# SKA-INAF/caesar-mrcnn

Hardware: AMD Instinct MI355X
Metric: train images/sec (whole node) + detect ms/image, ResNet-101 256x256 (higher is better)
Workload: dtype f32; 1 GPU; resnet101+FPN 256x256 3-class (+bg), nimg_per_gpu=4, train step (fwd+bwd+SGD), 512 train ROIs, 2000 proposals; global_batch=4, parallelism=dp1, weights=random init (Keras defaults)

## Files before the change

caesar-mrcnn_amd/_hip.py:

```python
import ctypes as C
import os
import threading

PKG_DIR = os.path.dirname(os.path.abspath(__file__))
LIB_PATH = os.path.join(PKG_DIR, "libmrcnn_hip.so")


class HipPathError(RuntimeError):
    pass


class ConvDesc(C.Structure):
    _fields_ = [(n, C.c_int32) for n in (
        "N", "H", "W", "Cin", "Cout", "KH", "KW", "stride", "pad_t", "pad_l", "OH", "OW",
        "act", "res_mode", "out_mode", "cmod")] + [
        ("out_n_stride", C.c_int64), ("out_h_stride", C.c_int64), ("out_w_stride", C.c_int64)]


class ConvProblem(C.Structure):
    _fields_ = [("d", ConvDesc)] + [(n, C.c_void_p) for n in ("x", "w", "bias", "scale", "shift", "res", "out", "z_out")]


class WgradProblem(C.Structure):
    _fields_ = [("d", ConvDesc), ("x", C.c_void_p), ("dy", C.c_void_p), ("dw", C.c_void_p), ("accumulate", C.c_int32)]
# ... 203 lines not shown
    "mrcnn_cast_to_h16": (C.c_int, [_P, _P, C.c_int64, C.c_int, C.c_float, _P]),
    "mrcnn_epilogue_bwd_h16": (C.c_int, [C.c_int] + [_P] * 10 + [C.c_int64, C.c_int, C.c_int, C.c_float, _P]),
    "mrcnn_epilogue_bwd_h16_dy": (C.c_int, [C.c_int] + [_P] * 11 + [C.c_int64, C.c_int, C.c_int, C.c_float, _P]),
    "mrcnn_cast_from_h16": (C.c_int, [_P, _P, C.c_int64, C.c_int, C.c_float, _P]),
    "mrcnn_axpy_from_h16": (C.c_int, [_P, _P, C.c_int64, C.c_int, C.c_float, _P]),
    "mrcnn_rpn_targets_workspace": (C.c_size_t, [C.POINTER(RpnTargetDesc)]),
    "mrcnn_rpn_targets": (C.c_int, [C.POINTER(RpnTargetDesc)] + [_P] * 7 + [C.c_size_t, _P]),
    "mrcnn_detection_workspace": (C.c_size_t, [C.POINTER(DetectionDesc)]),
    "mrcnn_detection_fwd": (C.c_int, [C.POINTER(DetectionDesc)] + [_P] * 6 + [C.c_size_t, _P]),
    "mrcnn_losses_workspace": (C.c_size_t, [C.POINTER(LossDesc)]),
    "mrcnn_losses_fwd_bwd": (C.c_int, [C.POINTER(LossDesc)] + [_P] * 18 + [C.c_size_t, _P]),
    "mrcnn_grad_prepare": (C.c_int, [_P, _P, C.c_float, _P, C.c_int64, _P, _P]),
    "mrcnn_sumsq": (C.c_int, [_P, C.c_int64, _P, _P]),
    "mrcnn_sgd_momentum": (C.c_int, [_P, _P, _P, _P, C.c_float, C.c_float, C.c_float, _P, C.c_int64, _P]),
    "mrcnn_sgd_momentum_guarded": (C.c_int, [_P, _P, _P, _P, C.c_float, C.c_float, C.c_float, _P, C.c_int64, _P, _P]),
    "mrcnn_winograd_buffer_floats": (C.c_size_t, [C.c_int, C.c_int, C.c_int, C.c_int, C.c_int]),
    "mrcnn_winograd_weights": (C.c_int, [_P, _P, C.c_int, C.c_int, C.c_int, _P]),
    "mrcnn_gemm_batched_f32": (C.c_int, [_P, _P, _P, C.c_int, C.c_int, C.c_int, C.c_int, _P]),
    "mrcnn_winograd_gemm": (C.c_int, [_P, _P, _P, C.c_int, C.c_int, C.c_int, C.c_int, _P]),
    "mrcnn_winograd_group_floats": (C.c_size_t, [C.POINTER(WinoGroup), C.c_int, C.c_int]),
    "mrcnn_winograd_input_g": (C.c_int, [_P, _P, C.c_int, C.c_int, C.c_int, C.c_int, C.POINTER(WinoGroup), _P]),
    "mrcnn_winograd_weights_g": (C.c_int, [_P, _P, C.c_int, C.c_int, C.c_int, C.c_int, _P]),
    "mrcnn_winograd_output_g": (C.c_int, [_P, _P, _P, _P, _P, _P, C.c_int, C.c_int, C.c_int, C.c_int, C.c_int, C.POINTER(WinoGroup), _P]),
    "mrcnn_winograd_output_bwd_rows": (C.c_int, [C.POINTER(WinoGroup), C.c_int, C.c_int]),
    "mrcnn_winograd_output_bwd_g": (C.c_int, [_P] * 8 + [C.c_int, C.c_int, C.c_int, C.c_int, C.c_int, C.POINTER(WinoGroup), _P]),
    "mrcnn_winograd_output_bwd_zmask_g": (C.c_int, [_P] * 8 + [C.c_int, C.c_int, C.c_int, C.c_int, C.POINTER(WinoGroup), _P]),
    "mrcnn_winograd_output_bwd_sums": (C.c_int, [_P, C.c_int, C.c_int, _P, _P, _P, _P]),
    "mrcnn_winograd_dy_g": (C.c_int, [_P, _P, C.c_int, C.c_int, C.c_int, C.c_int, C.POINTER(WinoGroup), _P]),
    "mrcnn_winograd_dw_g": (C.c_int, [_P, _P, C.c_int, C.c_int, C.c_int, C.c_int, C.c_int, _P]),
    "mrcnn_deconv2x2_gemm": (C.c_int, [_P, _P, _P, _P, C.c_int, C.c_int, C.c_int, C.c_int, C.c_int, C.c_int, _P]),
    "mrcnn_allreduce_load": (C.c_int, [C.c_char_p]),
    "mrcnn_allreduce_unique_id": (C.c_int, [_P]),
    "mrcnn_allreduce_init": (C.c_int, [C.POINTER(_P), _P, C.c_int, C.c_int]),
    "mrcnn_allreduce_scratch": (C.c_size_t, [C.c_int, C.c_int64, C.c_int]),
    "mrcnn_allreduce_grad": (C.c_int, [_P, _P, C.c_int64, C.c_int64, C.c_int, _P, C.c_size_t, _P]),
    "mrcnn_allreduce_direct_plan": (C.c_int, [C.c_int, C.c_int, C.c_int64, C.c_int64, C.c_int, _P, _P, _P, _P]),
    "mrcnn_allreduce_direct_simulate": (C.c_int, [_P, _P, C.c_size_t, C.c_int, C.c_int64, C.c_int64, _P]),
    "mrcnn_allreduce_destroy": (C.c_int, [_P]),
    "mrcnn_allreduce_last_error": (C.c_char_p, []),
    "mrcnn_tuning_set": (C.c_int, [C.c_char_p, C.c_longlong]),
    "mrcnn_hip_version": (C.c_char_p, []),
}

_lib = None
_proxy = None
_tape = None
# ... 119 lines not shown
```

caesar-mrcnn_amd/csrc/winograd.hip:

```cpp
#include "common.h"
#include <type_traits>
#include <string.h>

template <int CV> struct WinoVec;
template <> struct WinoVec<4> { typedef f32x4 type; };
template <> struct WinoVec<2> { typedef float type __attribute__((ext_vector_type(2))); };

template <int OT, typename V> __device__ __forceinline__ void wino_bt(const V (&d)[OT + 2], V (&t)[OT + 2]) {
    if constexpr (OT == 2) {
        t[0] = d[0] - d[2];
        t[1] = d[1] + d[2];
        t[2] = d[2] - d[1];
        t[3] = d[1] - d[3];
    } else {
        const V a = d[4] - 4.f * d[2], b = d[3] - 4.f * d[1], c = d[4] - d[2], e = 2.f * (d[3] - d[1]);
        t[0] = 4.f * d[0] - 5.f * d[2] + d[4];
        t[1] = a + b;
        t[2] = a - b;
        t[3] = c + e;
        t[4] = c - e;
        t[5] = 4.f * d[1] - 5.f * d[3] + d[5];
    }
}
template <int OT, typename V> __device__ __forceinline__ void wino_at(const V (&m)[OT + 2], V (&y)[OT]) {
// ... 181 lines not shown
    const long long t = i / cn;
    const int c = (int)(i - t * cn) * CV;
    vec bi = {}, sc, sh = {};
#pragma unroll
    for (int e = 0; e < CV; ++e) sc[e] = 1.f;
    if (bias) bi = *(const vec*)(bias + c);
    if (scale) { sc = *(const vec*)(scale + c); sh = *(const vec*)(shift + c); }
    wino_output_tile<OTH, OTW, CV>(Mt, out, z, bi, sc, sh, H, W, C, Tp, act, g, t, c);
}

template <int CV>
__device__ __forceinline__ typename WinoVec<CV>::type wino_buffer_load(__amdgpu_buffer_rsrc_t rsrc, unsigned voff, unsigned soff) {
    typename WinoVec<CV>::type r;
    if constexpr (CV == 2) {
        const auto v = __builtin_amdgcn_raw_buffer_load_b64(rsrc, (int)voff, (int)soff, 0);
        r[0] = __uint_as_float(v[0]); r[1] = __uint_as_float(v[1]);
    } else {
        const auto v = __builtin_amdgcn_raw_buffer_load_b128(rsrc, (int)voff, (int)soff, 0);
        r[0] = __uint_as_float(v[0]); r[1] = __uint_as_float(v[1]); r[2] = __uint_as_float(v[2]); r[3] = __uint_as_float(v[3]);
    }
    return r;
}

template <int OTH, int OTW, int CV, int MASK>
__global__ __launch_bounds__(256) void winograd_output_bwd_kernel(const float* __restrict__ Mt, float* __restrict__ dz_out,
                                                                  const float* __restrict__ below_out, const float* __restrict__ below_z,
                                                                  const float* __restrict__ scale, const float* __restrict__ mean,
                                                                  const float* __restrict__ rstd, const float* __restrict__ fwd_shift,
                                                                  float* __restrict__ partials, int want_dg, int H, int W, int C, unsigned T,
                                                                  long long Tp, int lg, const WinoGrp g, const FastDiv d_th,
                                                                  const FastDiv d_tw) {
    typedef typename WinoVec<CV>::type vec;
    constexpr int ITH = OTH + 2, ITW = OTW + 2;
    __shared__ float sacc[3 * 4 * 256];
    const int L = 1 << lg, R = 256 >> lg;
    const int rsub = threadIdx.x >> lg, lane = threadIdx.x & (L - 1);
    const int c = lane * CV;
    vec sc, mu = {}, rs = {}, fsh = {};
#pragma unroll
    for (int e = 0; e < CV; ++e) sc[e] = 1.f;
    if (scale) sc = *(const vec*)(scale + c);
    if (want_dg) { mu = *(const vec*)(mean + c); rs = *(const vec*)(rstd + c); }
    if (MASK == 1) fsh = *(const vec*)(fwd_shift + c);
    const bool need_z = MASK == 1 || want_dg;
    vec a_db = {}, a_dg = {}, a_bias = {};
    const unsigned step = gridDim.x * (unsigned)R;
// ... 366 lines not shown
    if (!x || !V || !wino_grp_ok(g, N, H, W, C)) return MRCNN_ERR_ARG;
    const long long T = wino_grp_tiles(g, N);
    const WinoGrp k = {g->th_n, g->tw_n, g->oh0, g->ow0};
    const dim3 g4((unsigned)cdiv64(T * C / 4, 256)), g2((unsigned)cdiv64(T * C / 2, 256));
    WINO_LAUNCH_G(winograd_input_kernel, g, g4, g2, x, V, N, H, W, C, T, wino_rows(T), k);
    return mrcnn_launch_status();
}

extern "C" int mrcnn_winograd_weights_g(const float* w, float* U, int Cin, int Cout, int oth, int otw, void* stream) {
    if (!w || !U || Cin <= 0 || Cout <= 0 || (oth != 2 && oth != 4) || (otw != 2 && otw != 4)) return MRCNN_ERR_ARG;
    const dim3 grid((unsigned)cdiv64((long long)Cin * Cout, 256));
    WINO_LAUNCH_W(winograd_weight_kernel, oth, otw, grid, w, U, Cin, Cout);
    return mrcnn_launch_status();
}

extern "C" int mrcnn_winograd_output_g(const float* Mt, float* out, float* z, const float* bias, const float* scale, const float* shift,
                                       int N, int H, int W, int C, int act, const mrcnn_wino_group* g, void* stream) {
    if (!Mt || !out || !wino_grp_ok(g, N, H, W, C) || (scale && !shift)) return MRCNN_ERR_ARG;
    if (act != MRCNN_ACT_NONE && act != MRCNN_ACT_RELU) return MRCNN_ERR_UNSUPPORTED;
    const long long T = wino_grp_tiles(g, N);
    const WinoGrp k = {g->th_n, g->tw_n, g->oh0, g->ow0};
    const dim3 g4((unsigned)cdiv64(T * C / 4, 256)), g2((unsigned)cdiv64(T * C / 2, 256));
    WINO_LAUNCH_G(winograd_output_kernel, g, g4, g2, Mt, out, z, bias, scale, shift, N, H, W, C, T, wino_rows(T), act, k);
    return mrcnn_launch_status();
}

static int wino_bwd_lanes_lg(const mrcnn_wino_group* g, int C) {
    const int cn = C / wino_grp_cv(g);
    if (cn <= 0 || cn > 256 || (cn & (cn - 1)) || cn * wino_grp_cv(g) != C) return -1;
    int lg = 0;
    while ((1 << lg) < cn) ++lg;
    return lg;
}
extern "C" int mrcnn_winograd_output_bwd_rows(const mrcnn_wino_group* g, int N, int C) {
    if (!g || N <= 0 || (g->oth != 2 && g->oth != 4) || (g->otw != 2 && g->otw != 4) || g->th_n <= 0 || g->tw_n <= 0) return 0;
    const int lg = wino_bwd_lanes_lg(g, C);
    if (lg < 0) return 0;
    const long long T = wino_grp_tiles(g, N), R = 256 >> lg, cap = 4LL * mrcnn_num_cus();
    const long long wgs = cdiv64(T, R);
    return (int)(wgs < cap ? wgs : cap);
}

template <int MASK>
static int wino_output_bwd_launch(const float* Mt, float* dz_below, const float* below_out, const float* below_z, const float* scale,
                                  const float* mean, const float* rstd, const float* fwd_shift, float* partials, int N, int H, int W,
                                  int C, const mrcnn_wino_group* g, void* stream) {
// ... 117 lines not shown
```

caesar-mrcnn_amd/engine.py:

```python
import collections
import contextlib
import gc
import operator
from functools import partial
import os
import numpy as np
import torch

from . import ops
from . import _hip as _hip_mod
from ._hip import ACT_NONE, ACT_RELU, ACT_SIGMOID, RES_NONE, RES_SAME, RES_UP2
from .params import ParamLayout, deconv_gemm_to_keras, deconv_keras_to_gemm, granule_coefficients, init_weights

H16_WIDE_LAYERS = ("fpn_p2", "fpn_p3", "fpn_p4", "fpn_p5", "rpn_conv_shared", "mrcnn_class_conv1", "mrcnn_class_conv2")

LOSS_NAMES = ("rpn_class_loss", "rpn_bbox_loss", "mrcnn_class_loss", "mrcnn_bbox_loss", "mrcnn_mask_loss")


DIRECT, WINO, H16 = "direct", "winograd", "h16"
Ctx = collections.namedtuple("Ctx", "x z out act path V", defaults=(DIRECT, None))
BlockCtx = collections.namedtuple("BlockCtx", "a b c shortcut h16")


_on = lambda s: s != "0"

SWITCHES = (
    ("head_dtype", None, None, None, "ti"),
    ("sparse_mask_bwd", None, True, None, "t"),
    ("h16_wide", "MRCNN_H16_WIDE", True, _on, "ti"),
    ("h16_blocks", "MRCNN_H16_BLOCKS", True, _on, "ti"),
    ("h16_all_blocks", "MRCNN_H16_ALL_BLOCKS", True, _on, "ti"),
    ("h16_fused_bwd", "MRCNN_H16_FUSED_BWD", True, _on, "t"),
    ("h16_roialign", "MRCNN_H16_ROIALIGN", True, _on, "ti"),
    ("h16_phase_bwd", "MRCNN_H16_PHASE_BWD", True, _on, "t"),
    ("winograd", "MRCNN_WINOGRAD", True, _on, "ti"),
    ("winograd_wgrad", "MRCNN_WINOGRAD_WGRAD", True, _on, "t"),
    ("trunk_winograd", "MRCNN_WINOGRAD_TRUNK", True, _on, "ti"),
    ("trunk_winograd_min_rows", "MRCNN_WINOGRAD_TRUNK_MIN_ROWS", 4096, int, "ti"),
    ("infer_mask_tile", "MRCNN_WINOGRAD_INFER_MASK_TILE", 4, int, "i"),
    ("sk16_infer", "MRCNN_SK16_INFER", True, _on, "i"),
    ("fused_mask_out_bwd", None, True, None, "t"),
    ("fused_dgrad_epilogue", None, True, None, "t"),
    ("gather_roialign_bwd", "MRCNN_GATHER_ROIALIGN_BWD", True, _on, "t"),
    ("multi_launch", "MRCNN_MULTI_LAUNCH", True, _on, "ti"),
    ("wgrad_prio", "MRCNN_WGRAD_PRIO", 0, int, ""),
    ("aux_prio", "MRCNN_AUX_PRIO", 0, int, ""),
)
_TRAIN_SWITCHES = operator.attrgetter(*(s[0] for s in SWITCHES if "t" in s[4]))
_INFER_SWITCHES = operator.attrgetter(*(s[0] for s in SWITCHES if "i" in s[4]))
_INFER_CFG = operator.attrgetter("PRE_NMS_LIMIT", "POST_NMS_ROIS_INFERENCE", "RPN_NMS_THRESHOLD", "DETECTION_MAX_INSTANCES",
                                 "DETECTION_MIN_CONFIDENCE", "DETECTION_NMS_THRESHOLD")


@contextlib.contextmanager
def _capture(graph):
    gc.collect()
    was = gc.isenabled()
    gc.disable()
    try:
# ... 387 lines not shown
        x16 = ca.x
        N, H, W, C = x16.shape
        st = c2a.stride
        dz1 = self._h16_bwd(blk.c1, dy, c1c, S, need_dx=False)
        dx = ops.empty((N, H, W, C), x16.dtype, x16.device)
        strides = None
        if st != 1:
            ops.fill_zero(dx)
            strides = (H * W * C, st * W * C, st * C)
        self._h16_dgrad(blk.c1, dz1, out=dx, out_strides=strides)
        self._h16_dgrad(c2a, dza, dx_res=dx, out=dx, out_strides=strides)
        return dx

    def _S(self):
        return float(self.loss_scale) if self.head_dtype == torch.float16 else 1.0

    def _wino_fwd(self, op, x, act, train, infer_tile=2):
        out = ops.empty(tuple(x.shape[:3]) + (op.wshape[3],), torch.float32, x.device)
        z = ops.empty_like(out) if (train and op.bn) else None
        V = ops.empty((ops.winograd_v_floats(tuple(x.shape)),), torch.float32, x.device) if (train and self.winograd_wgrad) else None
        ops.conv2d_winograd(x, self._wino_U(op, 0, x.shape, train, infer_tile), op.b, op.scale, op.shift, act, out=out, z_out=z, keep_v=V)
        return out, (Ctx(x, z, out, act, WINO, V) if train else None)

    def _forward_multi(self, layers, xs, act=ACT_NONE, train=False):
        if self.trunk_winograd and any(self._wino_trunk_ok(op, x.shape) for op, x in zip(layers, xs)):
            res = [None] * len(layers)
            rest = []
            for i, (op, x) in enumerate(zip(layers, xs)):
                if self._wino_trunk_ok(op, x.shape):
                    res[i] = self._wino_fwd(op, x, act, train)
                else:
                    rest.append(i)
            if rest:
                sub = self._forward_multi([layers[i] for i in rest], [xs[i] for i in rest], act, train) if len(rest) > 1 else \
                    [layers[rest[0]].forward(xs[rest[0]], act, train=train)]
                for i, r in zip(rest, sub):
                    res[i] = r
            return res
        if self.multi_launch and 1 < len(layers) <= 5:
            probs, zs = [], []
            for op, x in zip(layers, xs):
                d = ops.conv_desc(tuple(x.shape), op.wshape, op.stride, op.padding, act)
                out = ops.empty((d.N, d.OH, d.OW, d.Cout), torch.float32, x.device)
                z = ops.empty_like(out) if (train and op.bn) else None
                zs.append(z)
                probs.append(dict(x=x, w=op.w, bias=op.b, scale=op.scale, shift=op.shift, stride=op.stride,
# ... 237 lines not shown
                x16 = ops.cast_to_h16(x, self.head_dtype)
            h1, c1 = self._h16_fwd(self.op("mrcnn_class_conv1"), x16, ACT_RELU, train)
            h2_16, c2 = self._h16_fwd(self.op("mrcnn_class_conv2"), h1, ACT_RELU, train)
            h2 = ops.cast_from_h16(h2_16)
        else:
            h1, c1 = self.op("mrcnn_class_conv1").forward(x, ACT_RELU, train=train)
            h2, c2 = self.op("mrcnn_class_conv2").forward(h1, ACT_RELU, train=train)
        lg, c3 = self.op("mrcnn_class_logits").forward(h2, train=train)
        bb, c4 = self.op("mrcnn_bbox_fc").forward(h2, train=train)
        logits = lg.view(B, R, cfg.NUM_CLASSES)
        probs = ops.softmax_rows(logits)
        return logits, probs, bb.view(B, R, cfg.NUM_CLASSES, 4), (c1, c2, c3, c4)

    def _mask_head_fwd(self, rois, fms, p16h, image_area, train):
        cfg = self.cfg
        B, R = rois.shape[0], rois.shape[1]
        if p16h is not None:
            x = None
            x16 = ops.roialign_h16(rois, p16h, cfg.MASK_POOL_SIZE, image_area).view(B * R, cfg.MASK_POOL_SIZE, cfg.MASK_POOL_SIZE, -1)
        else:
            pooled = ops.roialign(rois, fms, cfg.MASK_POOL_SIZE, image_area)
            x = pooled.view(B * R, cfg.MASK_POOL_SIZE, cfg.MASK_POOL_SIZE, -1)
        ctxs = []
        if self.head_dtype is None:
            for i in range(1, 5):
                op = self.op("mrcnn_mask_conv%d" % i)
                if self._wino_ok(op, x.shape):
                    x, c = self._wino_fwd(op, x, ACT_RELU, train, self.infer_mask_tile)
                else:
                    x, c = op.forward(x, ACT_RELU, train=train)
                ctxs.append(c)
        else:
            self._ensure_h16()
            h = x16 if p16h is not None else ops.cast_to_h16(x, self.head_dtype)
            for i in range(1, 5):
                h, c = self._h16_fwd(self.op("mrcnn_mask_conv%d" % i), h, ACT_RELU, train)
                ctxs.append(c)
            dc, mop = self.op("mrcnn_mask_deconv"), self.op("mrcnn_mask")
            Cd = dc.wshape[3] // 4
            C_ = mop.wshape[3]
            if Cd % 256 == 0 and C_ <= 16:
                up = ops.deconv2x2_h16(h, self._h16[dc.name][0], dc.b, Cd, ACT_RELU)
                m = ops.mask_out_fwd_h16(up, mop.w.view(mop.wshape[2], C_), mop.b)
                ctxs.append(Ctx(h, None, up, ACT_RELU, H16) if train else None)
                ctxs.append(Ctx(up, None, m, ACT_SIGMOID, H16) if train else None)
                return m.view(B, R, m.shape[1], m.shape[2], m.shape[3]), ctxs
            x = ops.cast_from_h16(h)
# ... 167 lines not shown
        if cdec.path == H16:
            dzg = ops.mask_out_bwd_h16(g, cm.out, up, mop.w.view(mop.wshape[2], mop.wshape[3]),
                                       mop.dw.view(mop.wshape[2], mop.wshape[3]), mop.db, dc.db, S)
            wgrad(partial(ops.conv2d_wgrad_h16, x_in, dzg, dc.wshape, 1, "same", dw=dc.dw, multiplier=1.0 / S), x_in, dzg)
            d16 = ops.conv2d_h16(dzg, self._h16[dc.name][1], (1, 1, dc.wshape[3], dc.wshape[2]), None, None, None, 1, "valid",
                                 ACT_NONE)
        elif self.fused_mask_out_bwd and C_ <= 16 and up.shape[-1] % 64 == 0 and up.shape[-1] <= 1024:
            dzg = ops.mask_out_bwd(g, cm.out, up, mop.w.view(mop.wshape[2], mop.wshape[3]),
                                   mop.dw.view(mop.wshape[2], mop.wshape[3]), mop.db, dc.db)
        else:
            dz, _ = mop.epilogue_bwd(g, cm)
            mop.wgrad(dz, cm)
            d_up = mop.dgrad(dz, cm)
            dzu = ops.empty_like(d_up)
            ops.epilogue_bwd(d_up, up, None, None, None, None, None, dzu, None, None, dc.db, ACT_RELU)
            dzg = ops.pixel_unshuffle2(dzu)
        if d16 is None:
            wgrad(partial(ops.conv2d_wgrad, x_in, dzg, dc.wshape, 1, "valid", dw=dc.dw), x_in, dzg)
        chain = [(self.op("mrcnn_mask_conv%d" % i), c) for i, c in ((4, c4), (3, c3), (2, c2), (1, c1))]
        if c4.path != H16:
            dz = self._dgrad_ep(dzg, dc.wt, "valid", chain[0][0], chain[0][1])
            for k, (op, c) in enumerate(chain):
                if c.V is not None:
                    wgrad(partial(ops.conv2d_wgrad_winograd, c.V, tuple(c.x.shape), dz, op.dw), c.V, dz)
                else:
                    wgrad(partial(ops.conv2d_wgrad, c.x, dz, op.wshape, op.stride, op.padding, dw=op.dw), c.x, dz)
                wino = c.path == WINO
                if k + 1 < len(chain):
                    below, bctx = chain[k + 1]
                    if wino and self.fused_dgrad_epilogue and below.bn is not None:
                        dz = ops.conv2d_dgrad_ep_winograd(dz, self._wino_U(op, 1, dz.shape), bctx.out if bctx.act != ACT_NONE else None,
                                                          bctx.z, below.scale, below.mean, below.rstd, below.dgamma, below.dbeta,
                                                          below.db, bctx.act, fwd_shift=below.shift)
                    elif wino:
                        dz = below.epilogue_bwd(ops.conv2d_winograd(dz, self._wino_U(op, 1, dz.shape)), bctx)[0]
                    else:
                        dz = self._dgrad_ep(dz, op.wt, op.dgrad_padding, below, bctx)
                elif wino:
                    d = ops.conv2d_winograd(dz, self._wino_U(op, 1, dz.shape))
                else:
                    d = op.dgrad(dz, c)
        else:
            if d16 is None:
                d = ops.conv2d(dzg, dc.wt, stride=1, padding="valid")
                d16 = ops.cast_to_h16(d, self.head_dtype, multiplier=S)
            for op, c in chain:
                d16 = self._h16_bwd(op, d16, c, S)
# ... 315 lines not shown
```

caesar-mrcnn_amd/ops.py:

```python
import ctypes as C
import math
import os

import torch

from . import _hip
from ._hip import (ACT_NONE, ACT_RELU, ACT_SIGMOID, OUT_DECONV2, OUT_NHWC, RES_NONE, RES_SAME, RES_UP2,
                   check, current_stream, ptr)

BN_EPS = 1e-3


def _need_cuda(*ts):
    for t in ts:
        if t is not None and not t.is_cuda:
            raise _hip.HipPathError("hot-path operators need device tensors (got a CPU tensor)")
        if t is not None and not t.is_contiguous():
            raise _hip.HipPathError("hot-path operators need contiguous tensors")


def same_padding(size, k, stride):
    out = -(-size // stride)
    total = max((out - 1) * stride + k - size, 0)
    return out, total // 2
# ... 1710 lines not shown


def winograd_weights(w, out=None, tile=2):
    kh, kw, cin, cout = w.shape
    assert kh == 3 and kw == 3 and w.is_contiguous()
    if tile != TILE_MIXED:
        _need_cuda(w, out)
        nb = (tile + 2) ** 2
        if out is None:
            out = torch.empty((nb, cin, cout), dtype=torch.float32, device=w.device)
        assert out.shape[0] == nb
        check(_hip.lib().mrcnn_winograd_weights(ptr(w), ptr(out), cin, cout, tile, current_stream()), "mrcnn_winograd_weights")
        return out
    shapes = ((4, 4), (4, 2), (2, 4), (2, 2))
    if out is None:
        out = [torch.empty(((a + 2) * (b + 2), cin, cout), dtype=torch.float32, device=w.device) for a, b in shapes]
    _need_cuda(w, *out)
    for (a, b), u in zip(shapes, out):
        assert u.shape[0] == (a + 2) * (b + 2)
        check(_hip.lib().mrcnn_winograd_weights_g(ptr(w), ptr(u), cin, cout, a, b, current_stream()), "mrcnn_winograd_weights_g")
    return out


def _winograd_run(x, U, finish, keep_v=None, after_input=None):
    N, H, W, Cin = x.shape
    tile = _wino_tile_of(U)
    Us = U if isinstance(U, (list, tuple)) else [U]
    cout = Us[0].shape[2]
    groups = winograd_groups(H, W, tile)
    lib = _hip.lib()
    nvs = [lib.mrcnn_winograd_group_floats(C.byref(g), N, Cin) for g in groups]
    nms = [lib.mrcnn_winograd_group_floats(C.byref(g), N, cout) for g in groups]
    nv = sum(nvs)
    V = keep_v if keep_v is not None else workspace(nv * 4, x.device, "winograd_v")[:nv * 4].view(torch.float32)
    assert keep_v is None or (keep_v.numel() == nv and keep_v.dtype == torch.float32)
    Mt = workspace(max(nms) * 4, x.device, "winograd_m")
    off = 0
    for gi, (g, u) in enumerate(zip(groups, Us)):
        Vg = V[off:off + nvs[gi]]
        off += nvs[gi]
        check(lib.mrcnn_winograd_input_g(ptr(x), ptr(Vg), N, H, W, Cin, C.byref(g), current_stream()), "mrcnn_winograd_input_g")
        if gi == 0 and after_input is not None:
            after_input()
        nb = _wino_nb(g)
        rows = nvs[gi] // (nb * Cin)
        check(lib.mrcnn_winograd_gemm(ptr(Vg), ptr(u), ptr(Mt), nb, rows, Cin, cout, current_stream()), "mrcnn_winograd_gemm")
        finish(g, Mt)


def winograd_v_floats(xshape, tile=None):
    N, H, W, Cin = xshape
    if tile is None:
        tile = winograd_tile(xshape)
    lib = _hip.lib()
    return sum(lib.mrcnn_winograd_group_floats(C.byref(g), N, Cin) for g in winograd_groups(H, W, tile))


def conv2d_winograd(x, U, bias=None, scale=None, shift=None, act=ACT_NONE, out=None, z_out=None, keep_v=None, after_input=None):
    _need_cuda(x, bias, scale, shift, out, z_out, keep_v)
    N, H, W, _ = x.shape
    cout = (U[0] if isinstance(U, (list, tuple)) else U).shape[2]
    if out is None:
        out = empty((N, H, W, cout), torch.float32, x.device)
    lib = _hip.lib()

    def finish(g, Mt):
        check(lib.mrcnn_winograd_output_g(ptr(Mt), ptr(out), ptr(z_out), ptr(bias), ptr(scale), ptr(shift), N, H, W, cout, act, C.byref(g),
                                          current_stream()), "mrcnn_winograd_output_g")

    _winograd_run(x, U, finish, keep_v, after_input)
    return out


def conv2d_dgrad_ep_winograd(dz, Ut, below_out, below_z, scale, mean, rstd, dgamma, dbeta, dbias, act, fwd_shift=None):
    _need_cuda(dz, below_out, below_z, scale, mean, rstd, dgamma, dbeta, dbias, fwd_shift)
    N, H, W, _ = dz.shape
    cout = (Ut[0] if isinstance(Ut, (list, tuple)) else Ut).shape[2]
    out = empty((N, H, W, cout), torch.float32, dz.device)
    lib = _hip.lib()
    zmask = act == ACT_RELU and fwd_shift is not None and below_z is not None and scale is not None
    if dgamma is None:
        mean = rstd = None
    want_sums = dgamma is not None or dbeta is not None or dbias is not None
    rows = [lib.mrcnn_winograd_output_bwd_rows(C.byref(g), N, cout) for g in winograd_groups(H, W, _wino_tile_of(Ut))]
    assert min(rows) > 0, "channel count does not fit the Winograd data-gradient transform"
    part = ptr(workspace(sum(rows) * 3 * cout * 4, dz.device, "winograd_bwd_sums")) if want_sums else None
    done = []

    def finish(g, Mt):
        p = None
        if want_sums:
            p = part + sum(done) * 3 * cout * 4
            done.append(rows[len(done)])
        if zmask:
# ... 213 lines not shown
```

include/mrcnn_hip.h:

```cpp
#ifndef MRCNN_HIP_H
#define MRCNN_HIP_H

#include <stddef.h>
#include <stdint.h>

#ifdef __cplusplus
extern "C" {
#endif

#define MRCNN_OK 0
#define MRCNN_ERR_ARG (-1)
#define MRCNN_ERR_LAUNCH (-2)
#define MRCNN_ERR_WORKSPACE (-3)
#define MRCNN_ERR_UNSUPPORTED (-4)

#define MRCNN_ACT_NONE 0
#define MRCNN_ACT_RELU 1
#define MRCNN_ACT_SIGMOID 2

#define MRCNN_RES_NONE 0
#define MRCNN_RES_SAME 1
#define MRCNN_RES_UP2 2

#define MRCNN_OUT_NHWC 0
// ... 449 lines not shown
                       int64_t n, float* sumsq_out, void* stream);
int mrcnn_sumsq(const float* g, int64_t n, float* out_scalar, void* stream);
int mrcnn_sgd_momentum(float* params, float* momentum_buf, const float* grads, const float* sumsq,
                       float clipnorm, float lr, float momentum, const float* gran_coef, int64_t n,
                       void* stream);
int mrcnn_sgd_momentum_guarded(float* params, float* momentum_buf, const float* grads, const float* sumsq,
                               float clipnorm, float lr, float momentum, const float* gran_coef, int64_t n,
                               unsigned* skipped_steps, void* stream);

typedef struct mrcnn_wino_group {
    int oth, otw;
    int th_n, tw_n;
    int oh0, ow0;
} mrcnn_wino_group;
size_t mrcnn_winograd_group_floats(const mrcnn_wino_group* g, int N, int C);
size_t mrcnn_winograd_buffer_floats(int N, int H, int W, int C, int tile);
int mrcnn_winograd_weights(const float* w_hwio, float* U, int Cin, int Cout, int tile, void* stream);
int mrcnn_winograd_weights_g(const float* w_hwio, float* U, int Cin, int Cout, int oth, int otw, void* stream);
int mrcnn_winograd_input_g(const float* x, float* V, int N, int H, int W, int C, const mrcnn_wino_group* g, void* stream);
int mrcnn_gemm_batched_f32(const float* V, const float* U, float* Mt, int nb, int rows, int K, int Cout, void* stream);
int mrcnn_winograd_gemm(const float* V, const float* U, float* Mt, int nb, int rows, int K, int Cout, void* stream);
int mrcnn_winograd_output_g(const float* Mt, float* out, float* z_out, const float* bias, const float* scale, const float* shift,
                            int N, int H, int W, int C, int act, const mrcnn_wino_group* g, void* stream);
int mrcnn_winograd_output_bwd_rows(const mrcnn_wino_group* g, int N, int C);
int mrcnn_winograd_output_bwd_g(const float* Mt, float* dz_below, const float* below_out, const float* below_z, const float* scale,
                                const float* mean, const float* rstd, float* partials, int N, int H, int W, int C, int act,
                                const mrcnn_wino_group* g, void* stream);
int mrcnn_winograd_output_bwd_zmask_g(const float* Mt, float* dz_below, const float* below_z, const float* scale, const float* shift,
                                      const float* mean, const float* rstd, float* partials, int N, int H, int W, int C,
                                      const mrcnn_wino_group* g, void* stream);
int mrcnn_winograd_output_bwd_sums(const float* partials, int rows, int C, float* dgamma, float* dbeta, float* dbias, void* stream);
int mrcnn_winograd_dy_g(const float* dy, float* dM, int N, int H, int W, int C, const mrcnn_wino_group* g, void* stream);
int mrcnn_winograd_dw_g(const float* dU, float* dw_hwio, int Cin, int Cout, int accumulate, int oth, int otw, void* stream);

int mrcnn_deconv2x2_gemm(const float* x, const float* w_gemm, const float* bias, float* out, int N, int H, int W, int Cin, int Cd,
                         int act, void* stream);

#define MRCNN_UNIQUE_ID_BYTES 128
#define MRCNN_ALLREDUCE_RCCL 0
#define MRCNN_ALLREDUCE_DIRECT 1
int mrcnn_allreduce_load(const char* librccl_path);
int mrcnn_allreduce_unique_id(void* id_128_bytes);
int mrcnn_allreduce_init(void** comm, const void* id_128_bytes, int rank, int world);
size_t mrcnn_allreduce_scratch(int world, int64_t max_range_floats, int algo);
int mrcnn_allreduce_grad(void* comm, float* grads, int64_t start, int64_t end, int algo, float* scratch,
                         size_t scratch_bytes, void* stream);
// ... 25 lines not shown
```

Measured before the change: 115.8 images/s.

## Fuse Winograd output and next-layer input transforms in mask head chain

Adds a chained Winograd kernel for the training mask-head conv stack. It applies the output transform with bias/BN/ReLU into an LDS-resident feature map and then computes the next layer's Winograd input transform straight from LDS. This avoids writing the activation map to global memory and reading it back, and drops one kernel launch per layer. The next layer reuses the precomputed V, and the pre-activation z output is kept for backward. The Mt workspace now holds all tile groups at once, and the kernel needs large shared memory per block, which may lower occupancy.

```diff
diff --git a/caesar-mrcnn_amd/_hip.py b/caesar-mrcnn_amd/_hip.py
--- a/caesar-mrcnn_amd/_hip.py
+++ b/caesar-mrcnn_amd/_hip.py
@@ -249,6 +249,7 @@
     "mrcnn_winograd_input_g": (C.c_int, [_P, _P, C.c_int, C.c_int, C.c_int, C.c_int, C.POINTER(WinoGroup), _P]),
     "mrcnn_winograd_weights_g": (C.c_int, [_P, _P, C.c_int, C.c_int, C.c_int, C.c_int, _P]),
     "mrcnn_winograd_output_g": (C.c_int, [_P, _P, _P, _P, _P, _P, C.c_int, C.c_int, C.c_int, C.c_int, C.c_int, C.POINTER(WinoGroup), _P]),
+    "mrcnn_winograd_chain": (C.c_int, [_P] * 6 + [C.c_int] * 6 + [_P]),
     "mrcnn_winograd_output_bwd_rows": (C.c_int, [C.POINTER(WinoGroup), C.c_int, C.c_int]),
     "mrcnn_winograd_output_bwd_g": (C.c_int, [_P] * 8 + [C.c_int, C.c_int, C.c_int, C.c_int, C.c_int, C.POINTER(WinoGroup), _P]),
     "mrcnn_winograd_output_bwd_zmask_g": (C.c_int, [_P] * 8 + [C.c_int, C.c_int, C.c_int, C.c_int, C.POINTER(WinoGroup), _P]),
diff --git a/caesar-mrcnn_amd/csrc/winograd.hip b/caesar-mrcnn_amd/csrc/winograd.hip
--- a/caesar-mrcnn_amd/csrc/winograd.hip
+++ b/caesar-mrcnn_amd/csrc/winograd.hip
@@ -227,6 +227,139 @@
     return r;
 }
 
+struct WinoChainGeo {
+    int a, b;
+    unsigned tp[4];
+    long long off[4];
+};
+
+template <int OTH, int OTW>
+__device__ __forceinline__ void wino_chain_out_tile(__amdgpu_buffer_rsrc_t rsrc, unsigned mstride, unsigned t, int oh0, int ow0, int c,
+                                                    int cl, const WinoVec<2>::type bi, const WinoVec<2>::type sc,
+                                                    const WinoVec<2>::type sh, int act, float* __restrict__ z, float* map, int W,
+                                                    int C, int CS) {
+    typedef WinoVec<2>::type vec;
+    constexpr int ITH = OTH + 2, ITW = OTW + 2;
+    vec m[ITH][ITW];
+    const unsigned moff = (t * (unsigned)C + (unsigned)c) * 4u;
+#pragma unroll
+    for (int r = 0; r < ITH; ++r)
+#pragma unroll
+        for (int k = 0; k < ITW; ++k) m[r][k] = wino_buffer_load<2>(rsrc, moff, (unsigned)(r * ITW + k) * mstride);
+    vec s[OTH][ITW];
+#pragma unroll
+    for (int k = 0; k < ITW; ++k) {
+        vec col[ITH], o[OTH];
+#pragma unroll
+        for (int r = 0; r < ITH; ++r) col[r] = m[r][k];
+        wino_at<OTH>(col, o);
+#pragma unroll
+        for (int a = 0; a < OTH; ++a) s[a][k] = o[a];
+    }
+#pragma unroll
+    for (int a = 0; a < OTH; ++a) {
+        vec y[OTW];
+        wino_at<OTW>(s[a], y);
+#pragma unroll
+        for (int b = 0; b < OTW; ++b) {
+            const int pix = (oh0 + a) * W + ow0 + b;
+            vec zv, o;
+#pragma unroll
+            for (int e = 0; e < 2; ++e) {
+                zv[e] = y[b][e] + bi[e];
+                float v = sc[e] * zv[e] + sh[e];
+                if (act == MRCNN_ACT_RELU) v = fmaxf(v, 0.f);
+                o[e] = v;
+            }
+            if (z) *(vec*)(z + (unsigned)(pix * C + c)) = zv;
+            *(vec*)(map + pix * CS + cl) = o;
+        }
+    }
+}
+
+template <int OTH, int OTW>
+__device__ __forceinline__ void wino_chain_in_tile(const float* map, float* __restrict__ Vg, long long Tp, unsigned t, int oh0, int ow0, int c,
+                                                   int cl, int H, int W, int C, int CS) {
+    typedef WinoVec<2>::type vec;
+    constexpr int ITH = OTH + 2, ITW = OTW + 2;
+    const int ih0 = oh0 - 1, iw0 = ow0 - 1;
+    vec tt[ITH][ITW];
+#pragma unroll
+    for (int s = 0; s < ITW; ++s) {
+        vec col[ITH], o[ITH];
+#pragma unroll
+        for (int r = 0; r < ITH; ++r) {
+            const int ih = ih0 + r, iw = iw0 + s;
+            vec val = {};
+            if ((unsigned)ih < (unsigned)H && (unsigned)iw < (unsigned)W) val = *(const vec*)(map + (ih * W + iw) * CS + cl);
+            col[r] = val;
+        }
+        wino_bt<OTH>(col, o);
+#pragma unroll
+        for (int r = 0; r < ITH; ++r) tt[r][s] = o[r];
+    }
+#pragma unroll
+    for (int r = 0; r < ITH; ++r) {
+        vec v[ITW];
+        wino_bt<OTW>(tt[r], v);
+#pragma unroll
+        for (int s = 0; s < ITW; ++s) *(vec*)(Vg + ((long long)(r * ITW + s) * Tp + t) * C + c) = v[s];
+    }
+}
+
+__global__ __launch_bounds__(256, 3) void winograd_chain_kernel(const float* __restrict__ Mt, float* __restrict__ z, const float* __restrict__ bias,
+                                                             const float* __restrict__ scale, const float* __restrict__ shift,
+                                                             float* __restrict__ V, int H, int W, int C, int act, int lg,
+                                                             const WinoChainGeo geo) {
+    typedef WinoVec<2>::type vec;
+    extern __shared__ __attribute__((aligned(16))) float wino_chain_map[];
+    const int L = 1 << lg, CS = 2 << lg, slots = 256 >> lg;
+    const int slices = C / CS;
+    const int n = (int)(blockIdx.x / (unsigned)slices), slice = (int)(blockIdx.x - (unsigned)n * slices);
+    const int slot = threadIdx.x >> lg, cl = (threadIdx.x & (L - 1)) * 2;
+    const int c = slice * CS + cl;
+    const int a = geo.a, b = geo.b, n0 = a * b, per_map = n0 + a + b + 1;
+    vec bi = {}, sc, sh = {};
+    sc[0] = sc[1] = 1.f;
+    if (bias) bi = *(const vec*)(bias + c);
+    if (scale) { sc = *(const vec*)(scale + c); sh = *(const vec*)(shift + c); }
+    const __amdgpu_buffer_rsrc_t r0 = __builtin_amdgcn_make_buffer_rsrc((void*)(Mt + geo.off[0]), 0, 0xFFFFFFF0u, 0x00020000);
+    const __amdgpu_buffer_rsrc_t r1 = __builtin_amdgcn_make_buffer_rsrc((void*)(Mt + geo.off[1]), 0, 0xFFFFFFF0u, 0x00020000);
+    const __amdgpu_buffer_rsrc_t r2 = __builtin_amdgcn_make_buffer_rsrc((void*)(Mt + geo.off[2]), 0, 0xFFFFFFF0u, 0x00020000);
+    const __amdgpu_buffer_rsrc_t r3 = __builtin_amdgcn_make_buffer_rsrc((void*)(Mt + geo.off[3]), 0, 0xFFFFFFF0u, 0x00020000);
+    const unsigned cb = (unsigned)C * 4u;
+    float* zn = z ? z + (long long)n * H * W * C : nullptr;
+    for (int it = slot; it < per_map; it += slots) {
+        if (it < n0) {
+            const int th = it / b, tw = it - th * b;
+            wino_chain_out_tile<4, 4>(r0, geo.tp[0] * cb, (unsigned)n * n0 + it, 4 * th, 4 * tw, c, cl, bi, sc, sh, act, zn, wino_chain_map, W, C, CS);
+        } else if (it < n0 + a) {
+            const int th = it - n0;
+            wino_chain_out_tile<4, 2>(r1, geo.tp[1] * cb, (unsigned)n * a + th, 4 * th, W - 2, c, cl, bi, sc, sh, act, zn, wino_chain_map, W, C, CS);
+        } else if (it < n0 + a + b) {
+            const int tw = it - n0 - a;
+            wino_chain_out_tile<2, 4>(r2, geo.tp[2] * cb, (unsigned)n * b + tw, H - 2, 4 * tw, c, cl, bi, sc, sh, act, zn, wino_chain_map, W, C, CS);
+        } else {
+            wino_chain_out_tile<2, 2>(r3, geo.tp[3] * cb, (unsigned)n, H - 2, W - 2, c, cl, bi, sc, sh, act, zn, wino_chain_map, W, C, CS);
+        }
+    }
+    __syncthreads();
+    for (int it = slot; it < per_map; it += slots) {
+        if (it < n0) {
+            const int th = it / b, tw = it - th * b;
+            wino_chain_in_tile<4, 4>(wino_chain_map, V + geo.off[0], geo.tp[0], (unsigned)n * n0 + it, 4 * th, 4 * tw, c, cl, H, W, C, CS);
+        } else if (it < n0 + a) {
+            const int th = it - n0;
+            wino_chain_in_tile<4, 2>(wino_chain_map, V + geo.off[1], geo.tp[1], (unsigned)n * a + th, 4 * th, W - 2, c, cl, H, W, C, CS);
+        } else if (it < n0 + a + b) {
+            const int tw = it - n0 - a;
+            wino_chain_in_tile<2, 4>(wino_chain_map, V + geo.off[2], geo.tp[2], (unsigned)n * b + tw, H - 2, 4 * tw, c, cl, H, W, C, CS);
+        } else {
+            wino_chain_in_tile<2, 2>(wino_chain_map, V + geo.off[3], geo.tp[3], (unsigned)n, H - 2, W - 2, c, cl, H, W, C, CS);
+        }
+    }
+}
+
 template <int OTH, int OTW, int CV, int MASK>
 __global__ __launch_bounds__(256) void winograd_output_bwd_kernel(const float* __restrict__ Mt, float* __restrict__ dz_out,
                                                                   const float* __restrict__ below_out, const float* __restrict__ below_z,
@@ -639,6 +772,40 @@
     const WinoGrp k = {g->th_n, g->tw_n, g->oh0, g->ow0};
     const dim3 g4((unsigned)cdiv64(T * C / 4, 256)), g2((unsigned)cdiv64(T * C / 2, 256));
     WINO_LAUNCH_G(winograd_output_kernel, g, g4, g2, Mt, out, z, bias, scale, shift, N, H, W, C, T, wino_rows(T), act, k);
+    return mrcnn_launch_status();
+}
+
+static int wino_chain_slice(int H, int W) {
+    for (int cs = 64; cs >= 8; cs >>= 1)
+        if ((long long)H * W * cs * 4 <= 53 * 1024) return cs;
+    return (long long)H * W * 8 * 4 <= 64 * 1024 ? 8 : 0;
+}
+
+extern "C" int mrcnn_winograd_chain(const float* Mt, float* z_out, const float* bias, const float* scale, const float* shift, float* V_next,
+                                    int N, int H, int W, int C, int act, int tile, void* stream) {
+    if (!Mt || !V_next || N <= 0 || H <= 0 || W <= 0 || C <= 0 || (scale && !shift)) return MRCNN_ERR_ARG;
+    if (act != MRCNN_ACT_NONE && act != MRCNN_ACT_RELU) return MRCNN_ERR_UNSUPPORTED;
+    if (tile != MRCNN_WINO_TILE_MIXED || H % 4 != 2 || W % 4 != 2 || H <= 4 || W <= 4 || C % 128) return MRCNN_ERR_UNSUPPORTED;
+    const int cs = wino_chain_slice(H, W);
+    if (!cs) return MRCNN_ERR_UNSUPPORTED;
+    WinoChainGeo geo;
+    geo.a = H / 4; geo.b = W / 4;
+    const long long tiles[4] = {(long long)N * geo.a * geo.b, (long long)N * geo.a, (long long)N * geo.b, N};
+    const int nb[4] = {36, 24, 24, 16};
+    long long off = 0;
+    for (int i = 0; i < 4; ++i) {
+        const long long tp = wino_rows(tiles[i]);
+        if (tiles[i] >= (1LL << 31) || nb[i] * tp * C * 4 >= (1LL << 32)) return MRCNN_ERR_UNSUPPORTED;
+        geo.tp[i] = (unsigned)tp;
+        geo.off[i] = off;
+        off += nb[i] * tp * C;
+    }
+    const long long wgs = (long long)N * (C / cs);
+    if (wgs >= (1LL << 31)) return MRCNN_ERR_UNSUPPORTED;
+    int lg = 0;
+    while ((2 << lg) < cs) ++lg;
+    hipLaunchKernelGGL(winograd_chain_kernel, dim3((unsigned)wgs), dim3(256), (size_t)H * W * cs * 4, (hipStream_t)stream, Mt, z_out, bias, scale,
+                       shift, V_next, H, W, C, act, lg, geo);
     return mrcnn_launch_status();
 }
 
diff --git a/caesar-mrcnn_amd/engine.py b/caesar-mrcnn_amd/engine.py
--- a/caesar-mrcnn_amd/engine.py
+++ b/caesar-mrcnn_amd/engine.py
@@ -35,6 +35,7 @@
     ("h16_phase_bwd", "MRCNN_H16_PHASE_BWD", True, _on, "t"),
     ("winograd", "MRCNN_WINOGRAD", True, _on, "ti"),
     ("winograd_wgrad", "MRCNN_WINOGRAD_WGRAD", True, _on, "t"),
+    ("winograd_chain", "MRCNN_WINOGRAD_CHAIN", True, _on, "t"),
     ("trunk_winograd", "MRCNN_WINOGRAD_TRUNK", True, _on, "ti"),
     ("trunk_winograd_min_rows", "MRCNN_WINOGRAD_TRUNK_MIN_ROWS", 4096, int, "ti"),
     ("infer_mask_tile", "MRCNN_WINOGRAD_INFER_MASK_TILE", 4, int, "i"),
@@ -468,6 +469,40 @@
         ops.conv2d_winograd(x, self._wino_U(op, 0, x.shape, train, infer_tile), op.b, op.scale, op.shift, act, out=out, z_out=z, keep_v=V)
         return out, (Ctx(x, z, out, act, WINO, V) if train else None)
 
+    def _wino_link_ok(self, op, nxt, xshape):
+        tile = ops.winograd_tile(tuple(xshape))
+        oshape = tuple(xshape[:3]) + (op.wshape[3],)
+        return (self.winograd_chain and self.winograd_wgrad and self.fused_dgrad_epilogue and op.bn is not None and
+                tile == ops.TILE_MIXED and ops.winograd_chain_ok(tuple(xshape), op.wshape[3], tile) and
+                self._wino_ok(nxt, oshape) and ops.winograd_tile(oshape) == tile)
+
+    def _wino_chained_fwd(self, layers, x, act):
+        ctxs = []
+        shape, V = tuple(x.shape), None
+        for i, op in enumerate(layers):
+            if V is None and not self._wino_ok(op, shape):
+                x, c = op.forward(x, act, train=True)
+                ctxs.append(c)
+                shape = tuple(x.shape)
+                continue
+            nxt = layers[i + 1] if i + 1 < len(layers) else None
+            oshape = shape[:3] + (op.wshape[3],)
+            ready = V is not None
+            U = self._wino_U(op, 0, shape)
+            z = ops.empty(oshape, torch.float32, self.dev) if op.bn else None
+            if not ready and self.winograd_wgrad:
+                V = ops.empty((ops.winograd_v_floats(shape),), torch.float32, self.dev)
+            if nxt is not None and self._wino_link_ok(op, nxt, shape):
+                Vn = ops.empty((ops.winograd_v_floats(oshape),), torch.float32, self.dev)
+                out = ops.conv2d_winograd_chain(shape if ready else x, U, Vn, op.b, op.scale, op.shift, act, z_out=z, keep_v=V, v_ready=ready)
+            else:
+                Vn = None
+                out = ops.empty(oshape, torch.float32, self.dev)
+                ops.conv2d_winograd(shape if ready else x, U, op.b, op.scale, op.shift, act, out=out, z_out=z, keep_v=V, v_ready=ready)
+            ctxs.append(Ctx(x, z, out, act, WINO, V))
+            x, shape, V = out, oshape, Vn
+        return x, ctxs
+
     def _forward_multi(self, layers, xs, act=ACT_NONE, train=False):
         if self.trunk_winograd and any(self._wino_trunk_ok(op, x.shape) for op, x in zip(layers, xs)):
             res = [None] * len(layers)
@@ -751,7 +786,9 @@
             pooled = ops.roialign(rois, fms, cfg.MASK_POOL_SIZE, image_area)
             x = pooled.view(B * R, cfg.MASK_POOL_SIZE, cfg.MASK_POOL_SIZE, -1)
         ctxs = []
-        if self.head_dtype is None:
+        if self.head_dtype is None and train:
+            x, ctxs = self._wino_chained_fwd([self.op("mrcnn_mask_conv%d" % i) for i in range(1, 5)], x, ACT_RELU)
+        elif self.head_dtype is None:
             for i in range(1, 5):
                 op = self.op("mrcnn_mask_conv%d" % i)
                 if self._wino_ok(op, x.shape):
@@ -965,7 +1002,7 @@
             dz = self._dgrad_ep(dzg, dc.wt, "valid", chain[0][0], chain[0][1])
             for k, (op, c) in enumerate(chain):
                 if c.V is not None:
-                    wgrad(partial(ops.conv2d_wgrad_winograd, c.V, tuple(c.x.shape), dz, op.dw), c.V, dz)
+                    wgrad(partial(ops.conv2d_wgrad_winograd, c.V, tuple(dz.shape[:3]) + (op.wshape[2],), dz, op.dw), c.V, dz)
                 else:
                     wgrad(partial(ops.conv2d_wgrad, c.x, dz, op.wshape, op.stride, op.padding, dw=op.dw), c.x, dz)
                 wino = c.path == WINO
diff --git a/caesar-mrcnn_amd/ops.py b/caesar-mrcnn_amd/ops.py
--- a/caesar-mrcnn_amd/ops.py
+++ b/caesar-mrcnn_amd/ops.py
@@ -1756,8 +1756,9 @@
     return out
 
 
-def _winograd_run(x, U, finish, keep_v=None, after_input=None):
-    N, H, W, Cin = x.shape
+def _winograd_run(x, U, finish, keep_v=None, after_input=None, v_ready=False, finish_all=None):
+    N, H, W, Cin = x if v_ready else x.shape
+    assert not v_ready or keep_v is not None
     tile = _wino_tile_of(U)
     Us = U if isinstance(U, (list, tuple)) else [U]
     cout = Us[0].shape[2]
@@ -1766,20 +1767,27 @@
     nvs = [lib.mrcnn_winograd_group_floats(C.byref(g), N, Cin) for g in groups]
     nms = [lib.mrcnn_winograd_group_floats(C.byref(g), N, cout) for g in groups]
     nv = sum(nvs)
-    V = keep_v if keep_v is not None else workspace(nv * 4, x.device, "winograd_v")[:nv * 4].view(torch.float32)
+    dev = Us[0].device
+    V = keep_v if keep_v is not None else workspace(nv * 4, dev, "winograd_v")[:nv * 4].view(torch.float32)
     assert keep_v is None or (keep_v.numel() == nv and keep_v.dtype == torch.float32)
-    Mt = workspace(max(nms) * 4, x.device, "winograd_m")
-    off = 0
+    Mt = workspace((max(nms) if finish_all is None else sum(nms)) * 4, dev, "winograd_m")
+    off = moff = 0
     for gi, (g, u) in enumerate(zip(groups, Us)):
         Vg = V[off:off + nvs[gi]]
         off += nvs[gi]
-        check(lib.mrcnn_winograd_input_g(ptr(x), ptr(Vg), N, H, W, Cin, C.byref(g), current_stream()), "mrcnn_winograd_input_g")
+        if not v_ready:
+            check(lib.mrcnn_winograd_input_g(ptr(x), ptr(Vg), N, H, W, Cin, C.byref(g), current_stream()), "mrcnn_winograd_input_g")
         if gi == 0 and after_input is not None:
             after_input()
         nb = _wino_nb(g)
         rows = nvs[gi] // (nb * Cin)
-        check(lib.mrcnn_winograd_gemm(ptr(Vg), ptr(u), ptr(Mt), nb, rows, Cin, cout, current_stream()), "mrcnn_winograd_gemm")
-        finish(g, Mt)
+        check(lib.mrcnn_winograd_gemm(ptr(Vg), ptr(u), ptr(Mt) + moff * 4, nb, rows, Cin, cout, current_stream()), "mrcnn_winograd_gemm")
+        if finish_all is None:
+            finish(g, Mt)
+        else:
+            moff += nms[gi]
+    if finish_all is not None:
+        finish_all(Mt)
 
 
 def winograd_v_floats(xshape, tile=None):
@@ -1790,20 +1798,62 @@
     return sum(lib.mrcnn_winograd_group_floats(C.byref(g), N, Cin) for g in winograd_groups(H, W, tile))
 
 
-def conv2d_winograd(x, U, bias=None, scale=None, shift=None, act=ACT_NONE, out=None, z_out=None, keep_v=None, after_input=None):
-    _need_cuda(x, bias, scale, shift, out, z_out, keep_v)
-    N, H, W, _ = x.shape
-    cout = (U[0] if isinstance(U, (list, tuple)) else U).shape[2]
+def conv2d_winograd(x, U, bias=None, scale=None, shift=None, act=ACT_NONE, out=None, z_out=None, keep_v=None, after_input=None,
+                    v_ready=False):
+    _need_cuda(None if v_ready else x, bias, scale, shift, out, z_out, keep_v)
+    N, H, W, _ = x if v_ready else x.shape
+    U0 = U[0] if isinstance(U, (list, tuple)) else U
+    cout = U0.shape[2]
     if out is None:
-        out = empty((N, H, W, cout), torch.float32, x.device)
+        out = empty((N, H, W, cout), torch.float32, U0.device)
     lib = _hip.lib()
 
     def finish(g, Mt):
         check(lib.mrcnn_winograd_output_g(ptr(Mt), ptr(out), ptr(z_out), ptr(bias), ptr(scale), ptr(shift), N, H, W, cout, act, C.byref(g),
                                           current_stream()), "mrcnn_winograd_output_g")
 
-    _winograd_run(x, U, finish, keep_v, after_input)
-    return out
+    _winograd_run(x, U, finish, keep_v, after_input, v_ready)
+    return out
+
+
+def winograd_chain_ok(xshape, cout, tile):
+    _, H, W, _ = xshape
+    return tile == TILE_MIXED and H % 4 == 2 and W % 4 == 2 and H > 4 and W > 4 and cout % 128 == 0 and H * W <= 2048
+
+
+def conv2d_winograd_chain(x, U, next_v, bias=None, scale=None, shift=None, act=ACT_NONE, z_out=None, keep_v=None, v_ready=False):
+    _need_cuda(None if v_ready else x, bias, scale, shift, z_out, keep_v, next_v)
+    N, H, W, _ = x if v_ready else x.shape
+    Us = U if isinstance(U, (list, tuple)) else [U]
+    cout = Us[0].shape[2]
+    tile = _wino_tile_of(U)
+    groups = winograd_groups(H, W, tile)
+    lib = _hip.lib()
+    nms = [lib.mrcnn_winograd_group_floats(C.byref(g), N, cout) for g in groups]
+    assert next_v.numel() == sum(nms) and next_v.dtype == torch.float32
+    res = []
+
+    def finish_all(Mt):
+        rc = lib.mrcnn_winograd_chain(ptr(Mt), ptr(z_out), ptr(bias), ptr(scale), ptr(shift), ptr(next_v), N, H, W, cout, act, tile,
+                                      current_stream())
+        if rc != ERR_UNSUPPORTED:
+            check(rc, "mrcnn_winograd_chain")
+            return
+        out = empty((N, H, W, cout), torch.float32, next_v.device)
+        off = 0
+        for g, nm in zip(groups, nms):
+            check(lib.mrcnn_winograd_output_g(ptr(Mt) + off * 4, ptr(out), ptr(z_out), ptr(bias), ptr(scale), ptr(shift), N, H, W, cout, act,
+                                              C.byref(g), current_stream()), "mrcnn_winograd_output_g")
+            off += nm
+        off = 0
+        for g, nm in zip(groups, nms):
+            check(lib.mrcnn_winograd_input_g(ptr(out), ptr(next_v) + off * 4, N, H, W, cout, C.byref(g), current_stream()),
+                  "mrcnn_winograd_input_g")
+            off += nm
+        res.append(out)
+
+    _winograd_run(x, U, None, keep_v, None, v_ready, finish_all)
+    return res[0] if res else None
 
 
 def conv2d_dgrad_ep_winograd(dz, Ut, below_out, below_z, scale, mean, rstd, dgamma, dbeta, dbias, act, fwd_shift=None):
diff --git a/include/mrcnn_hip.h b/include/mrcnn_hip.h
--- a/include/mrcnn_hip.h
+++ b/include/mrcnn_hip.h
@@ -495,6 +495,9 @@
 int mrcnn_winograd_gemm(const float* V, const float* U, float* Mt, int nb, int rows, int K, int Cout, void* stream);
 int mrcnn_winograd_output_g(const float* Mt, float* out, float* z_out, const float* bias, const float* scale, const float* shift,
                             int N, int H, int W, int C, int act, const mrcnn_wino_group* g, void* stream);
+#define MRCNN_WINO_TILE_MIXED 6
+int mrcnn_winograd_chain(const float* Mt, float* z_out, const float* bias, const float* scale, const float* shift, float* V_next,
+                         int N, int H, int W, int C, int act, int tile, void* stream);
 int mrcnn_winograd_output_bwd_rows(const mrcnn_wino_group* g, int N, int C);
 int mrcnn_winograd_output_bwd_g(const float* Mt, float* dz_below, const float* below_out, const float* below_z, const float* scale,
                                 const float* mean, const float* rstd, float* partials, int N, int H, int W, int C, int act,
```

Measured after the change: 117.1 images/s (median of 6 runs). 1.01x the previous value.
